# JacobMackay/beifong

Hardware: AMD Instinct MI355X
Metric: Mrays/s (closest + any-hit BVH queries), Bus.obj-class radar scene (higher is better)
Workload: dtype f32

## Files before the change

### beifong_amd/csrc/bf_api.cpp

```cpp
#include <hip/hip_runtime.h>

#include <algorithm>
#include <atomic>
#include <cmath>
#include <cstdarg>
#include <cstdio>
#include <cstring>
#include <limits>
#include <memory>
#include <new>
#include <string>
#include <vector>

#include <dlfcn.h>
#if defined(__has_include) && __has_include(<rccl/rccl.h>)
#include <rccl/rccl.h>
#else
extern "C" {
typedef struct ncclComm *ncclComm_t;
typedef enum { ncclSuccess = 0 } ncclResult_t;
typedef enum { ncclFloat = 7 } ncclDataType_t;
typedef enum { ncclSum = 0 } ncclRedOp_t;
ncclResult_t ncclCommInitAll(ncclComm_t *comm, int ndev, const int *devlist);
ncclResult_t ncclCommDestroy(ncclComm_t comm);
// ... 2616 lines not shown
        if (launch->flags & BF_FLAG_MIX_RESAMPLE) return fail(BF_ERR_INVALID, "BF_FLAG_MIX_RESAMPLE is a receive-mode flag");
        if (is_rx) return fail(BF_ERR_INVALID, "render modes need a sensor (fluxmeter / perspective), not a receiver");
        for (uint32_t i = 0; i < scene->d.n_emitters; ++i)
            if (scene->emitter_types[i] != BF_EMITTER_SPOT && scene->emitter_types[i] != BF_EMITTER_AREA &&
                scene->emitter_types[i] != BF_EMITTER_POINT)
                return fail(BF_ERR_INVALID, "render modes: emitter %u is a transmitter (use receive mode)", i);
    }
    if (launch->mode > BF_MODE_RECEIVE_IQ) return fail(BF_ERR_INVALID, "unknown mode %u", launch->mode);
    if (launch->mode != BF_MODE_RECEIVE_RAW && launch->phase_bins)
        return fail(BF_ERR_INVALID, "phase_bins needs receive mode (PhaseIntegrator wraps pathtimefrequency)");
    if (launch->phase_bins > 4096) return fail(BF_ERR_INVALID, "phase_bins %u out of range", launch->phase_bins);
    if ((launch->mode == BF_MODE_RANGE || launch->mode == BF_MODE_TIME) && (launch->bins == 0 || !(launch->bin_width > 0.f)))
        return fail(BF_ERR_INVALID, "range/time mode needs bins > 0 and bin_width > 0");
    const bool multi_pixel = launch->spp && launch->film_width && launch->film_height;
    if (multi_pixel ? (launch->film_width != scene->film_w || launch->film_height != scene->film_h)
                    : (scene->film_w != 1 || scene->film_h != 1) && !is_rx)
        return fail(BF_ERR_INVALID, "the sensor's film is %u x %u: the launch must name the same film and spp > 0 (it has %u x %u, spp %u)",
                    scene->film_w, scene->film_h, launch->film_width, launch->film_height, launch->spp);
    if (multi_pixel) {
        if (launch->mode == BF_MODE_RECEIVE_RAW || launch->mode == BF_MODE_RECEIVE_IQ)
            return fail(BF_ERR_INVALID, "receive modes bin into the ADC: film_width / film_height / spp must be 0");
        const uint64_t px = (uint64_t) launch->film_width * launch->film_height;
        if (px > (1u << 24) || px * (5ull + 3ull * launch->bins) > (1ull << 31))
            return fail(BF_ERR_UNSUPPORTED, "film %u x %u with %u bins is too large", launch->film_width, launch->film_height, launch->bins);
        if (launch->path_offset + launch->n_paths > px * launch->spp)
            return fail(BF_ERR_INVALID, "path_offset + n_paths = %llu exceeds film_width * film_height * spp = %llu",
                        (unsigned long long) (launch->path_offset + launch->n_paths), (unsigned long long) (px * launch->spp));
    }
    if ((launch->flags & BF_FLAG_MOMENT) && (launch->flags & BF_FLAG_FAST))
        return fail(BF_ERR_INVALID, "BF_FLAG_MOMENT | BF_FLAG_FAST: the fast-arithmetic tolerance contract says nothing about squared "
                                    "samples; render second moments with the exact kernels");
    if (multi_pixel && (launch->flags & BF_FLAG_MOMENT) && (uint64_t) launch->film_width * launch->film_height * (11ull + 6ull * launch->bins) > (1ull << 31))
        return fail(BF_ERR_UNSUPPORTED, "film %u x %u with %u bins and BF_FLAG_MOMENT is too large", launch->film_width, launch->film_height, launch->bins);
    hipStream_t stream = reinterpret_cast<hipStream_t>(stream_);
    const bool rolling = (launch->flags & BF_FLAG_ROLLING) != 0u && launch->n_paths != 0u &&
                         (uint64_t) n_renders * launch->n_paths <= scene->tun.pool && n_renders <= bfd::kRollRing;
    if (launch->flags & BF_FLAG_ROLLING) {
        if (scene->roll.open && ((launch->flags ^ scene->roll.shape.flags) & BF_FLAG_FAST))
            return fail(BF_ERR_INVALID, "BF_FLAG_ROLLING: the open rolling sequence of this handle was started %s BF_FLAG_FAST; "
                                        "flush it (bf_scene_flush) before rolling renders of the other mode",
                        (scene->roll.shape.flags & BF_FLAG_FAST) ? "with" : "without");
        if (scene->roll.open && ((launch->flags ^ scene->roll.shape.flags) & BF_FLAG_MOMENT))
            return fail(BF_ERR_INVALID, "BF_FLAG_ROLLING: the open rolling sequence of this handle was started %s BF_FLAG_MOMENT; "
                                        "flush it (bf_scene_flush) before rolling renders of the other layout",
                        (scene->roll.shape.flags & BF_FLAG_MOMENT) ? "with" : "without");
        if (multi_pixel || (launch->flags & BF_FLAG_MEGAKERNEL))
            return fail(BF_ERR_UNSUPPORTED, "BF_FLAG_ROLLING: multi-pixel films and the one-kernel variant do not roll");
        if (stats_out)
            return fail(BF_ERR_INVALID, "BF_FLAG_ROLLING: a rolling render returns before its paths have ended, so it has no statistics "
                                        "of its own (pass stats_out = NULL; bf_scene_flush reports the sequence's)");
    }
    {
        bf_status ost = order_after_last(scene, stream);
        if (ost != BF_OK) return ost;
        if (!rolling && (ost = close_sequence(scene, stream)) != BF_OK) return ost;
    }
    bfd::DLaunch lp;
    std::memset(&lp, 0, sizeof(lp));
    lp.film_w = multi_pixel ? launch->film_width : 1u;
    lp.film_h = multi_pixel ? launch->film_height : 1u;
    lp.spp = multi_pixel ? launch->spp : 0u;
    lp.mode = launch->mode;
    lp.color_mode = launch->color_mode;
    lp.n_paths = launch->n_paths;
    lp.path_offset = launch->path_offset;
    lp.seed = launch->seed;
    lp.max_depth = launch->max_depth;
    lp.rr_depth = launch->rr_depth;
    lp.bins = launch->bins;
    lp.bins_y = launch->bins_y;
    lp.phase_bins = launch->mode == BF_MODE_RECEIVE_RAW ? launch->phase_bins : 0u;
    lp.iq = launch->mode == BF_MODE_RECEIVE_IQ ? 1u : 0u;
    if (lp.iq) lp.mode = BF_MODE_RECEIVE_RAW;
    lp.bin_width = launch->bin_width;
    lp.time_c = launch->time_c;
    lp.n_chan = bf_launch_channels(launch);
    lp.chan_px = lp.n_chan / (lp.film_w * lp.film_h);
    lp.lean = lean_profile(scene, launch, receive_mode, multi_pixel) ? 1u : 0u;
    lp.wide = scene->sensor_host.filt_n != 0u ? 1u : 0u;
    scene->last_variant = (lp.lean ? (uint32_t) BF_VARIANT_LEAN : 0u) | (lp.wide ? (uint32_t) BF_VARIANT_WIDE : 0u);
    if (launch->flags & BF_FLAG_FAST) scene->last_variant |= (uint32_t) BF_VARIANT_FAST;
    if (launch->flags & BF_FLAG_MOMENT) scene->last_variant |= (uint32_t) BF_VARIANT_MOMENT;
    const Kernels &kern = kernels_for(launch->flags);
    lp.count = ((launch->flags & (BF_FLAG_STATS | BF_FLAG_COUNT)) || stats_out) ? 1u : 0u;
    lp.doppler = (receive_mode && (launch->flags & BF_FLAG_DOPPLER)) ? 1u : 0u;
    lp.resample = (receive_mode && scene->any_resample) ? 1u : 0u;
    if (lp.resample && lp.doppler)
        return fail(BF_ERR_UNSUPPORTED, "BF_FLAG_DOPPLER with a resample_freq transmitter: both rewrite the path's wavelength (one slot of path state)");
    lp.mix = (receive_mode && (launch->flags & BF_FLAG_MIX_RESAMPLE)) ? 1u : 0u;
    lp.n_chan_all = lp.n_chan * n_renders;
    lp.geom_stride = geom_stride;
    lp.lds_hist = (lp.n_chan_all <= (uint32_t) bfd::kMaxLdsHist && !(launch->flags & BF_FLAG_GLOBAL_ATOMICS)) ? 1u : 0u;
    lp.lds_floats = lp.lds_hist ? lp.n_chan_all : 0u;
    size_t lds = sizeof(int) * bfd::kStackDepth * bfd::kBlock + (lp.lds_hist ? sizeof(float) * lp.n_chan_all : 0);
    lds = ((lds + 15) & ~size_t(15)) + (scene->d.tab_cache ? bfd::kTabBytes : 0u);
    if (batch && !rolling) {
        lp.batch = n_renders;
        lp.batch_paths = launch->n_paths;
        lp.n_paths = launch->n_paths * n_renders;
        const size_t seed_bytes = batch->seeds ? ((sizeof(uint64_t) * n_renders + 15) & ~size_t(15)) : 0;
        const size_t off_bytes = batch->mesh_offsets ? sizeof(float4) * n_renders : 0;
        if (seed_bytes + off_bytes) {
            bf_scene::Stage *stg = nullptr;
            bf_status sst = stage_acquire(scene, seed_bytes + off_bytes, &stg);
            if (sst != BF_OK) return sst;
            if (seed_bytes) {
                std::memcpy(stg->host, batch->seeds, sizeof(uint64_t) * n_renders);
                lp.batch_seeds = (const uint64_t *) stg->dev;
            }
            if (off_bytes) {
                float4 *o = (float4 *) ((char *) stg->host + seed_bytes);
                float dmax = 0.f;
                for (uint32_t k = 0; k < n_renders; ++k) {
                    const float *q = batch->mesh_offsets + 3 * k;
                    if (!(std::isfinite(q[0]) && std::isfinite(q[1]) && std::isfinite(q[2])))
                        return fail(BF_ERR_INVALID, "bf_render_batch: non-finite mesh offset of render %u", k);
                    o[k] = make_float4(q[0], q[1], q[2], 0.f);
                    dmax = std::max({dmax, std::fabs(q[0]), std::fabs(q[1]), std::fabs(q[2])});
                }
                if (scene->d.n_tris) {
                    lp.batch_offsets = (const float4 *) ((char *) stg->dev + seed_bytes);
                    lp.box_slack = 1e-6f * (scene->origin_scale_built + 2.f * dmax);
                }
            }
            sst = stage_commit(stg, seed_bytes + off_bytes, stream);
            if (sst != BF_OK) return sst;
        }
    }

    uint64_t want = (lp.n_paths + bfd::kBlock - 1) / bfd::kBlock;
    unsigned blocks_per_cu = (unsigned) std::max<size_t>(1, std::min<size_t>(4, (160 * 1024) / lds));
    unsigned grid = (unsigned) std::max<uint64_t>(1, std::min<uint64_t>(want, (uint64_t) scene->n_cus * blocks_per_cu));

    if (rolling) {
        bf_status rst = wf_roll_render(scene, launch, batch, lp, hist_dev, records_dev, stream);
        if (rst != BF_OK) return rst;
        return mark_last(scene, stream);
    }
    HIP_TRY(hipMemsetAsync(scene->counters, 0, sizeof(unsigned long long) * bfd::CTR_GUARD, stream));
    hipEvent_t ev0 = nullptr, ev1 = nullptr;
    if (stats_out) {
        HIP_TRY(hipEventCreate(&ev0));
        HIP_TRY(hipEventCreate(&ev1));
        HIP_TRY(hipEventRecord(ev0, stream));
    }
    if (launch->n_paths) {
        if (launch->flags & BF_FLAG_MEGAKERNEL) {
            HIP_TRY(kern.render(&scene->d, &lp, hist_dev, records_dev, scene->counters,
                                (launch->flags & BF_FLAG_STATS) ? 1 : 0, grid, lds, stream));
        } else {
            bf_status wst = wf_render(scene, kern, lp, hist_dev, records_dev, stream, (launch->flags & BF_FLAG_STATS) != 0,
                                      stats_out != nullptr);
            if (wst != BF_OK) return wst;
        }
    }
    if (stats_out) {
        HIP_TRY(hipEventRecord(ev1, stream));
        HIP_TRY(hipEventSynchronize(ev1));
        unsigned long long c[bfd::CTR_COUNT];
        HIP_TRY(hipMemcpy(c, scene->counters, sizeof(c), hipMemcpyDeviceToHost));
        if ((launch->flags & BF_FLAG_MEGAKERNEL) || !launch->n_paths) {
            scene->wf_ms[0] = scene->wf_ms[1] = scene->wf_ms[2] = 0.f;
            scene->wf_trace_launches = scene->wf_iters = scene->wf_tail_launches = scene->wf_shade_launches = 0;
        }
        fill_stats(scene, c, lp.n_paths, stats_out);
        float ms = 0.f;
        hipError_t he = hipEventElapsedTime(&ms, ev0, ev1);
// ... 289 lines not shown
                std::memcpy(o, to_world + 12 * r, 12 * sizeof(float));
                o[12] = moves[r] ? 1.f : 0.f;
                o[13] = o[14] = o[15] = 0.f;
            }
        if ((pst = stage_commit(stg, bytes, stream)) != BF_OK) return pst;
        HIP_TRY(bfk_launch_deform_tris(scene->geom->corners, (const bfd::DDeformSrc *) stg->dev, tris0, a + L.tris, normals0,
                                       scene->d.normals ? a + L.normals : nullptr, scene->d.n_tris,
                                       to_world ? (const float *) ((const char *) stg->dev + src_bytes) : nullptr, kc, L.rows, n_shapes * 16u,
                                       bound, scene->deform_bad, stream));
        HIP_TRY(hipEventRecord(stg->ev, stream));
        HIP_TRY(bfk_launch_refit(a + L.tris, nodes0, a + L.nodes, scene->d.qnodes ? a + L.qnodes : nullptr, scene->d.n_nodes, rf.lvl4,
                                 rf.off4.data(), (uint32_t) rf.off4.size() - 1u, a + L.ubox4, wnodes0, scene->d.wnodes ? a + L.wnodes : nullptr,
                                 rf.lvl16, rf.off16.data(), (uint32_t) rf.off16.size() - 1u, a + L.ubox16, 2e-7f * oscale, kc, L.rows, stream));
        return BF_OK;
    });
    if (st != BF_OK || !n_deform) return st;
    if ((st = deform_watch(scene, stream)) != BF_OK) return st;
    return stats_out ? deform_report(scene, true) : BF_OK;
}

bf_status bf_render_device(const bf_scene *scene, const bf_launch *launch, float *hist_dev, bf_path_record *records_dev,
                           void *stream, bf_stats *stats_out) {
    return render_common(scene, launch, nullptr, hist_dev, records_dev, stream, stats_out);
}

bf_status bf_render_batch_device(const bf_scene *scene, const bf_launch *launch, const bf_batch *batch, float *hist_dev,
                                 bf_path_record *records_dev, void *stream, bf_stats *stats_out) {
    if (!batch) return fail(BF_ERR_INVALID, "bf_render_batch_device: null batch");
    return render_common(scene, launch, batch, hist_dev, records_dev, stream, stats_out);
}

bf_status bf_scene_flush(bf_scene *scene, void *stream_, bf_stats *stats_out) {
    if (!scene) return fail(BF_ERR_INVALID, "null argument");
    BF_ENTER(scene);
    hipStream_t stream = reinterpret_cast<hipStream_t>(stream_);
    const bool was_open = scene->roll.open;
    const uint64_t n_paths = was_open ? scene->roll.lp.n_paths : 0;
    bf_status st = order_after_last(scene, stream);
    if (st != BF_OK) return st;
    if (was_open) {
        if ((st = wf_roll_flush(scene, stream, stats_out != nullptr)) != BF_OK) return st;
        if ((st = mark_last(scene, stream)) != BF_OK) return st;
    }
    if (stats_out) {
        std::memset(stats_out, 0, sizeof(*stats_out));
        if (!was_open) return BF_OK;
        HIP_TRY(hipStreamSynchronize(stream));
        unsigned long long c[bfd::CTR_COUNT];
        HIP_TRY(hipMemcpy(c, scene->counters, sizeof(c), hipMemcpyDeviceToHost));
        fill_stats(scene, c, n_paths, stats_out);
        stats_out->kernel_ms = scene->wf_ms[0] + scene->wf_ms[1] + scene->wf_ms[2];
        if (c[bfd::CTR_GUARD] || c[bfd::CTR_SURV_GUARD]) {
            HIP_TRY(hipMemset(scene->counters + bfd::CTR_GUARD, 0, 2 * sizeof(unsigned long long)));
            scene->wf_fb_pending = false;
            return wf_guard_error(c[bfd::CTR_GUARD], c[bfd::CTR_SURV_GUARD]);
        }
        return scene->roll.lp.count ? check_film_count(c, n_paths) : BF_OK;
    }
    return BF_OK;
}

bf_status bf_scene_sync(bf_scene *scene) {
    if (!scene) return fail(BF_ERR_INVALID, "null argument");
    BF_ENTER(scene);
    bf_status st = close_sequence(scene, scene->roll.stream);
    if (st != BF_OK) return st;
    if (scene->has_last) HIP_TRY(hipEventSynchronize(scene->last_done));
    scene->wf_fb_pending = false;
    scene->roll.fb_call_iters = 0;
    unsigned long long lost = 0, refused = 0;
    bf_status gst = read_guards(scene, &lost, &refused);
    if (gst != BF_OK) return gst;
    if (lost || refused) return wf_guard_error(lost, refused);
    return deform_report(scene, true);
}

bf_status bfdbg_preload_guard(bf_scene *scene, unsigned long long n) {
    if (!scene) return fail(BF_ERR_INVALID, "null argument");
    HIP_TRY(hipDeviceSynchronize());
    HIP_TRY(hipMemcpy(scene->counters + bfd::CTR_GUARD, &n, sizeof(n), hipMemcpyHostToDevice));
    return BF_OK;
}

extern "C" hipError_t bfk_gather_probe(int mode, const float4 *table, uint32_t n_rows, float4 *out, hipStream_t stream);
bf_status bfdbg_gather_probe(int mode, uint32_t log2_rows, uint32_t reps, float *ms_out) {
    if (mode < 0 || mode > 2 || log2_rows < 10 || log2_rows > 28 || reps == 0) return fail(BF_ERR_INVALID, "bfdbg_gather_probe: bad arguments");
    const uint32_t n = 1u << log2_rows;
    float4 *table = nullptr, *flush = nullptr, *out = nullptr;
    hipEvent_t e0 = nullptr, e1 = nullptr;
    hipError_t e = hipMalloc((void **) &table, (size_t) n * 16);
    if (e == hipSuccess) e = hipMalloc((void **) &flush, (size_t) n * 16);
    if (e == hipSuccess) e = hipMalloc((void **) &out, 1024 * 16);
    if (e == hipSuccess) e = hipMemset(table, 0, (size_t) n * 16);
    if (e == hipSuccess) e = hipMemset(flush, 0, (size_t) n * 16);
    if (e == hipSuccess) e = hipEventCreate(&e0);
    if (e == hipSuccess) e = hipEventCreate(&e1);
    float total = 0.f;
    for (uint32_t r = 0; r < reps && e == hipSuccess; ++r) {
        e = hipMemsetAsync(flush, (int) (r & 1u), (size_t) n * 16, nullptr);
        if (e == hipSuccess) e = hipEventRecord(e0, nullptr);
        if (e == hipSuccess) e = bfk_gather_probe(mode, table, n, out, nullptr);
        if (e == hipSuccess) e = hipEventRecord(e1, nullptr);
        if (e == hipSuccess) e = hipEventSynchronize(e1);
        float ms = 0.f;
        if (e == hipSuccess) e = hipEventElapsedTime(&ms, e0, e1);
        total += ms;
    }
    if (e0) (void) hipEventDestroy(e0);
    if (e1) (void) hipEventDestroy(e1);
    (void) hipFree(table);
    (void) hipFree(flush);
    (void) hipFree(out);
    if (e != hipSuccess) return fail(BF_ERR_DEVICE, "bfdbg_gather_probe: %s", hipGetErrorString(e));
    if (ms_out) *ms_out = total / (float) reps;
    return BF_OK;
}

bf_status bfdbg_hold_busy(bf_scene *scene, int on) {
    if (!scene) return fail(BF_ERR_INVALID, "null argument");
    if (on) {
        if (scene->busy.test_and_set(std::memory_order_acquire)) return fail(BF_ERR_INVALID, "bfdbg_hold_busy: already held");
    } else {
        scene->busy.clear(std::memory_order_release);
    }
    return BF_OK;
}


void bf_shard_range(uint64_t n_paths, uint32_t shard, uint32_t n_shards, uint64_t *offset, uint64_t *count) {
    if (n_shards == 0) n_shards = 1;
    auto cut = [&](uint64_t k) -> uint64_t { return (uint64_t) (((unsigned __int128) n_paths * k) / n_shards); };
    const uint64_t lo = cut(shard), hi = cut((uint64_t) shard + 1u);
    if (offset) *offset = lo;
    if (count) *count = hi - lo;
}

extern "C++" {
namespace {
struct Rccl {
    void *lib = nullptr;
    decltype(&ncclCommInitAll) comm_init_all = nullptr;
    decltype(&ncclCommDestroy) comm_destroy = nullptr;
    decltype(&ncclAllReduce) all_reduce = nullptr;
    decltype(&ncclGroupStart) group_start = nullptr;
    decltype(&ncclGroupEnd) group_end = nullptr;
    decltype(&ncclGetErrorString) error_string = nullptr;
    std::string why;
};
Rccl &rccl() {
    static Rccl r = [] {
        Rccl q;
        const char *forced = getenv("BF_RCCL_LIB");
        const char *names[] = {forced && *forced ? forced : "librccl.so.1", "librccl.so", "/opt/rocm/lib/librccl.so.1"};
        const size_t n_names = forced && *forced ? 1 : 3;
        for (size_t i = 0; i < n_names && !q.lib; ++i)
            q.lib = dlopen(names[i], RTLD_NOW | RTLD_NOLOAD | RTLD_LOCAL);
        std::string last;
        for (size_t i = 0; i < n_names && !q.lib; ++i) {
            q.lib = dlopen(names[i], RTLD_NOW | RTLD_LOCAL);
            if (!q.lib) {
                const char *e = dlerror();
                last = e ? e : "";
            }
        }
        if (!q.lib) {
            q.why = std::string(forced && *forced ? forced : "librccl.so") + " not found: " + last;
// ... 513 lines not shown
```

### beifong_amd/csrc/bf_device.h

```cpp
#pragma once
#include <hip/hip_runtime.h>

#include "bf_ns.h"
#include <stddef.h>
#include <stdint.h>

#include "../../include/beifong_hip.h"

BF_NS_BEGIN

constexpr uint32_t kTriStride = 3;
constexpr int kBlock = 256;
constexpr int kStackDepth = 32;
constexpr int kMaxLdsHist = 12288;
constexpr int kWideStack = 512;
constexpr uint32_t kTopNodes = 85;

struct DRect {
    float to_world[12];
    float to_object[12];
    float s[3], t[3], n[3];
    float inv_area;
    float area;
    uint32_t shape;
// ... 91 lines not shown

#define BF_CAS __attribute__((address_space(4)))
typedef const BF_CAS DRect CRect;
typedef const BF_CAS DShape CShape;
typedef const BF_CAS DEmitter CEmitter;
typedef const BF_CAS DSensor CSensor;
template <class T> __device__ __forceinline__ const BF_CAS T *as_const(const T *p) { return (const BF_CAS T *) (uintptr_t) p; }
__device__ __forceinline__ CRect *c_rects(const DScene &sc) { return as_const(sc.rects); }
__device__ __forceinline__ CShape *c_shapes(const DScene &sc) { return as_const(sc.shapes); }
__device__ __forceinline__ CEmitter *c_emitters(const DScene &sc) { return as_const(sc.emitters); }
__device__ __forceinline__ CSensor &c_sensor(const DScene &sc) { return *as_const(sc.sensor); }

struct DRoll {
    uint64_t seed, path_offset;
    float *hist;
    bf_path_record *records;
    const DRect *rects;
    const DShape *shapes;
    const DEmitter *emitters;
    const DMaterial *materials;
    const DSensor *sensor;
    float c, lambda_min, lambda_max;
    uint32_t pad;
};
static_assert(sizeof(DRoll) == 88, "descriptor ring entry");
struct DDeformSrc {
    const float *pos;
    const float *nrm;
    uint32_t nv;
    uint32_t pad;
};
static_assert(sizeof(DDeformSrc) == 24, "per-shape table of bf_deform_tris_kernel");

constexpr uint32_t kRollRing = 256;
constexpr uint32_t kRollWindow = 4;
constexpr uint32_t kRollBase = 32;
constexpr uint32_t kRollBaseCh = 5, kRollBaseChMoment = 11;

struct DLaunch {
    uint32_t mode, color_mode;
    uint64_t n_paths, path_offset, seed;
    int32_t max_depth, rr_depth;
    uint32_t bins, bins_y, phase_bins;
    float bin_width, time_c;
    uint32_t n_chan;
    uint32_t lds_hist;
    uint32_t iq;
    uint32_t film_w, film_h;
    uint32_t spp;
    uint32_t chan_px;
    uint32_t batch;
    uint32_t n_chan_all;
    uint64_t batch_paths;
    const uint64_t *batch_seeds;
    const float4 *batch_offsets;
    uint32_t mix;
    uint32_t doppler;
    uint32_t resample;
    float box_slack;
    const DRoll *roll;
    uint32_t roll_newest;
    uint32_t roll_lo;
    uint32_t lds_floats;
    uint32_t base_off;
    uint32_t has_records;
    uint32_t lean;
    uint32_t wide;
    uint32_t multi;
    uint32_t count;
    uint32_t geom_stride;
};

enum {
    CTR_NEXT_PATH = 0, CTR_CLOSEST, CTR_SHADOW, CTR_NODES, CTR_TRIS, CTR_INVALID, CTR_BOUNCES, CTR_TAIL_RAYS, CTR_STARTED, CTR_TRACED,
    CTR_NODES_LDS,
    CTR_TAIL_NODES,
    CTR_TAIL_WNODES,
    CTR_TAIL_TRIS,
    CTR_TAIL_BOUNCES,
    CTR_SHADE_LOADS,
    CTR_SHADE_STORES,
    CTR_SHADE_SHADOW,
    CTR_SHADE_RAYS,
    CTR_FILM,
    CTR_GUARD,
    CTR_SURV_GUARD,
    CTR_COUNT
};

BF_NS_END
```

### beifong_amd/csrc/bf_path_logic.h

```cpp
#pragma once
#include "bf_device_core.h"
#include "bf_wavefront.h"

BF_NS_BEGIN

constexpr uint32_t kFlagValid = 1u << 24, kFlagFilmOk = 1u << 25, kFlagTermPending = 1u << 26, kDepthMask = 0xffffffu;
constexpr uint32_t kFlagFilmLeft = 1u << 27, kFlagFilmUp = 1u << 28;

struct PathState {
    V3 ro, rd;
    float rmint, rmaxt;
    float throughput, eta, emission_weight, result;
    float aux, bs_pdf;
    V3 prev_p;
    uint32_t flags;
    uint32_t n_rays;
    Rng rng;
    uint64_t path_i;
    uint32_t render;
    float time;
    float t_rx;
    float lambda0;
    float phase;
    float dlambda;
};

BF_DEV void load_state(const WF &wf, uint32_t i, bool receive, PathState &s) {
    float4 r0 = wf.ray0(i), r1 = wf.ray1(i), a = wf.sa(i), bb = wf.sb(i);
    uint4 d = wf.sd(i);
    s.ro = mk(r0.x, r0.y, r0.z);
    s.rmint = r0.w;
    s.rd = mk(r1.x, r1.y, r1.z);
    s.rmaxt = r1.w;
    s.throughput = a.x;
    s.eta = a.y;
    s.emission_weight = a.z;
    s.result = a.w;
    s.aux = bb.x;
    s.bs_pdf = bb.y;
    s.prev_p = s.ro;
    s.flags = __float_as_uint(bb.z);
    s.n_rays = __float_as_uint(bb.w);
    s.rng.state = ((uint64_t) d.y << 32) | d.x;
    s.path_i = ((uint64_t) d.w << 32) | d.z;
    s.time = s.t_rx = s.lambda0 = s.phase = 0.f;
    s.render = wf.has_render ? wf.render(i) : 0u;
    s.dlambda = wf.has_dop ? wf.dop(i) : 0.f;
    if (receive) {
        float4 e = wf.se(i);
        s.time = e.x;
        s.t_rx = e.y;
        s.lambda0 = e.z;
        s.phase = e.w;
    }
}
BF_DEV void store_state(const WF &wf, uint32_t j, bool receive, const PathState &s) {
    wf.ray0(j) = make_float4(s.ro.x, s.ro.y, s.ro.z, s.rmint);
    wf.ray1(j) = make_float4(s.rd.x, s.rd.y, s.rd.z, s.rmaxt);
    wf.sa(j) = make_float4(s.throughput, s.eta, s.emission_weight, s.result);
    wf.sb(j) = make_float4(s.aux, s.bs_pdf, __uint_as_float(s.flags), __uint_as_float(s.n_rays));
    wf.sd(j) = make_uint4((uint32_t) s.rng.state, (uint32_t) (s.rng.state >> 32), (uint32_t) s.path_i,
                          (uint32_t) (s.path_i >> 32));
    if (receive) wf.se(j) = make_float4(s.time, s.t_rx, s.lambda0, s.phase);
    if (wf.has_render) wf.render(j) = s.render;
    if (wf.has_dop) wf.dop(j) = s.dlambda;
}
BF_DEV float shape_doppler(const DScene &sc, const SI &si, float lambda_nm) {
    V3 q = xf_point(c_shapes(sc)[si.shape].velocity, to_local(si.sh, si.p));
    return 2.f * dot(si.wi, q) / sc.c * lambda_nm;
}
template <int V> BF_DEV DScene path_scene(const DScene &sc, const DLaunch &lp, uint32_t render) {
    if (!(V & (kMulti | kGeom))) return sc;
    DScene r = sc;
    if (V & kMulti) {
        const BF_CAS DRoll &e = as_const(lp.roll)[render & (kRollRing - 1u)];
        r.rects = e.rects;
        r.shapes = e.shapes;
        r.emitters = e.emitters;
        r.materials = e.materials;
        r.sensor = e.sensor;
        r.c = e.c;
        r.lambda_min = e.lambda_min;
        r.lambda_max = e.lambda_max;
        r.tab_on = 0u;
    }
    if (V & kGeom) geom_version(r, (uint64_t) render * lp.geom_stride);
    return r;
}
BF_DEV Shift path_shift(const DLaunch &lp, uint32_t render) { return make_shift(lp.batch_offsets, render, lp.box_slack); }

BF_DEV uint32_t nth_set_bit(unsigned long long m, uint32_t r) {
    uint32_t pos = 0;
#pragma unroll
    for (int shift = 32; shift >= 1; shift >>= 1) {
        unsigned long long lowmask = (1ull << shift) - 1ull;
        uint32_t cnt = (uint32_t) __popcll(m & lowmask);
        if (r >= cnt) {
            r -= cnt;
            m >>= shift;
            pos += shift;
        } else {
            m &= lowmask;
        }
    }
    return pos;
}

struct MaskCursor {
    const unsigned long long *masks;
    const unsigned long long *masks2;
    uint32_t sel;
    uint32_t b, b_end;
    unsigned long long m;
    uint32_t base, stride;
    uint32_t k;
    unsigned long long sub;
    unsigned long long w;
    unsigned long long nz;
    uint32_t rot, mod, inv, pb;
};
BF_DEV unsigned long long wave_read_u64(unsigned long long v, int src) {
    unsigned lo = (unsigned) __shfl((int) (unsigned) v, src), hi = (unsigned) __shfl((int) (unsigned) (v >> 32), src);
    return ((unsigned long long) hi << 32) | lo;
}
BF_DEV void cursor_fetch(MaskCursor &c, int lane) {
    const uint32_t idx = c.base + (c.k * 64u + (uint32_t) lane) * c.stride;
    uint32_t p = idx + c.rot;
    if (p >= c.mod) p -= c.mod;
    c.w = 0ull;
    if (idx < c.b_end) {
        c.w = c.masks ? c.masks[p] : ~0ull;
        if (c.inv) c.w = ~c.w;
        c.w &= c.sub;
        if (c.sel) c.w &= c.sel == 1u ? c.masks2[p] : ~c.masks2[p];
    }
    c.nz = __ballot(c.w != 0ull);
}
BF_DEV void cursor_seek(MaskCursor &c, int lane) {
    while (true) {
        if (c.nz) {
            const int j = __ffsll((unsigned long long) c.nz) - 1;
            c.nz &= c.nz - 1ull;
            c.b = c.base + (c.k * 64u + (uint32_t) j) * c.stride;
// ... 395 lines not shown
    } while (0)
#else
#define BF_LANEPROF_ARG
#define SLP(sec, cond)
#endif
template <int RX = 2>
BF_DEV bool shade_vertex(const DScene &sc0, const DLaunch &lp, PathState &s, const Hit &hit, ShadowReq &sh,
                         uint32_t &c_bounces BF_SHADEPROF_ARG BF_LANEPROF_ARG) {
    BF_SHADEPROF_STAMP(spf_t0);
    const DScene sc = path_scene<RX>(sc0, lp, s.render);
    const bool receive = mode_receive<RX>(lp);
    const bool is_range = !receive && lp.mode == BF_MODE_RANGE, is_time = rare<RX>(!receive && lp.mode == BF_MODE_TIME);
    const bool iq = receive && lp.iq != 0u;
    const bool phase_bins = rare<RX>(receive && lp.phase_bins != 0u);
    const bool doppler = rare<RX>(receive && lp.doppler != 0u);
    const uint32_t n_emit = (RX & kLean) ? 1u : sc.n_emitters;
    sh.want = false;
    SI si;
    const bool si_valid = hit.t != BF_INF;
    int emitter = -1;
    SLP(10, si_valid);
    bf_material mat;
    mat.type = ~0u;
    mat.back_material = 0u;
    if (si_valid) {
        make_si<false, RX>(sc, s.ro, s.rd, hit, si, nullptr, path_shift(lp, s.render));
        emitter = si.emitter;
        mat = load_material(sc, si.material);
    }
#ifdef BF_VERTEX_PROF
    asm volatile("s_waitcnt vmcnt(0)" ::: "memory");
#endif
    BF_SHADEPROF_STAMP(spf_t1);
    uint32_t depth = s.flags & kDepthMask;
    if (depth == 0) {
        if (si_valid) s.flags |= kFlagValid;
        if (is_range) s.aux += si_valid ? si.t : 0.f;
        if (is_time) s.aux = si_valid ? si.t / lp.time_c : 0.f;
        if (si_valid && doppler) s.dlambda += shape_doppler(sc, si, s.lambda0);
        if (receive && si_valid) {
            s.time += -si.t / sc.c;
            if (phase_bins) s.phase = phase_update(s.phase, -si.t, sc.lambda_min, sc.lambda_max);
        }
        depth = 1;
    } else {
        if (receive) {
            s.time += -hit.t / sc.c;
            if (phase_bins) s.phase = phase_update(0.f, -hit.t, sc.lambda_min, sc.lambda_max);
        }
        SLP(11, emitter >= 0);
        if (emitter >= 0) {
            CEmitter &e = c_emitters(sc)[(RX & kLean) ? 0 : emitter];
            float emitter_pdf = receive ? transmitter_pdf_direction<RX>(sc, e, s.prev_p, si.p, si.sh.n, s.lambda0)
                                        : emitter_pdf_direction<RX>(sc, e, s.prev_p, si.p, si.sh.n);
            if (n_emit != 1) emitter_pdf *= 1.f / (float) n_emit;
            s.emission_weight = mis_weight(s.bs_pdf, emitter_pdf);
        }
        if (is_range) s.aux += si_valid ? si.t : 0.f;
        if (is_time) s.aux += si_valid ? si.t / lp.time_c : 0.f;
        ++depth;
    }
    s.flags = (s.flags & ~kDepthMask) | (depth & kDepthMask);
    SLP(12, emitter >= 0);
    if (emitter >= 0) {
        CEmitter &e = c_emitters(sc)[(RX & kLean) ? 0 : emitter];
        if (doppler) s.dlambda += shape_doppler(sc, si, s.lambda0);
        float ev;
        if (receive)
            ev = transmitter_eval<RX>(sc, e, si, s.time, s.lambda0);
        else
            ev = ((RX & kLean) || e.type == BF_EMITTER_AREA) ? ((si.wi.z > 0.f) ? e.radiance : 0.f) : 0.f;
        float contrib = s.emission_weight * s.throughput * ev;
        if (iq) {
            float re, im;
            path_phasor((s.t_rx - s.time) * sc.c, s.lambda0, re, im);
            s.result += contrib * re;
            s.phase += contrib * im;
        } else {
            s.result += contrib;
        }
        if (is_range) s.aux += si_valid ? si.t : 0.f;
    }
    bool active = si_valid;
    if ((int) depth > lp.rr_depth) {
        float q = __builtin_fminf(s.throughput * sqr(s.eta), .95f);
        active = (next_1d(s.rng) < q) && active;
        s.throughput *= rcp(q);
    }
    if (depth >= (uint32_t) lp.max_depth || !active) return false;

    if (rare<RX>(mat.back_material != 0u) && si.wi.z < 0.f) mat = load_material(sc, mat.back_material - 1u);
    ++c_bounces;
    BF_SHADEPROF_STAMP(spf_t2);
    SLP(13, true);
    SLP(15, mat.type == BF_BSDF_ROUGHCONDUCTOR);
    SLP(16, mat.type != BF_BSDF_ROUGHCONDUCTOR);
    if (bsdf_smooth(mat)) {
        float sx = next_1d(s.rng), sy = next_1d(s.rng);
        DirSample ds;
        ds.d = mk(0, 0, 1);
        ds.pdf = 0.f;
        ds.dist = 0.f;
        ds.delta = false;
        float emitter_val = 0.f;
        if (n_emit >= 1) {
            uint32_t index = 0;
            float emitter_pdf = 1.f;
            if (n_emit > 1) {
                emitter_pdf = 1.f / (float) n_emit;
                index = min((uint32_t) (sx * (float) n_emit), n_emit - 1u);
                sx = (sx - index * emitter_pdf) * (float) n_emit;
            }
            CEmitter &e = c_emitters(sc)[index];
            if (receive)
                emitter_val = transmitter_sample_direction<RX>(sc, e, si.p, s.time, s.lambda0, sx, sy, ds);
            else
                emitter_val = emitter_sample_direction<RX>(sc, e, si.p, sx, sy, ds);
            if (n_emit > 1) {
                ds.pdf *= emitter_pdf;
                emitter_val *= rcp(emitter_pdf);
            }
        }
        SLP(14, ds.pdf != 0.f);
        if (ds.pdf != 0.f) {
            V3 wo = to_local(si.sh, ds.d);
            float bsdf_val, bsdf_pdf;
            bsdf_eval_pdf(mat, si.wi, wo, bsdf_val, bsdf_pdf);
            float mis = ds.delta ? 1.f : mis_weight(ds.pdf, bsdf_pdf);
            sh.c = mis * s.throughput * bsdf_val * emitter_val;
            sh.c_im = 0.f;
            if (iq) {
                float re, im;
                path_phasor((s.t_rx - s.time) * sc.c + ds.dist, s.lambda0, re, im);
                sh.c_im = sh.c * im;
                sh.c = sh.c * re;
            }
            sh.o = si.p;
            sh.d = ds.d;
            sh.mint = kRayEpsilon * (1.f + hmax_abs(si.p));
            sh.maxt = ds.dist * (1.f - kShadowEpsilon);
            sh.want = true;
            ++s.n_rays;
        }
        if (is_range) s.aux += si.t;
    }
    BF_SHADEPROF_STAMP(spf_t3);
    (void) next_1d(s.rng);
    float s2x = next_1d(s.rng), s2y = next_1d(s.rng);
    BSDFSample bs;
    float bsdf_val = bsdf_sample(mat, si.wi, s2x, s2y, bs);
    s.throughput = s.throughput * bsdf_val;
    if (s.throughput == 0.f) {
        s.flags |= kFlagTermPending;
        s.rmint = BF_INF;
        s.rmaxt = 0.f;
        return true;
    }
    s.eta *= bs.eta;
    s.ro = si.p;
    s.rd = to_world(si.sh, bs.wo);
    s.rmint = (1.f + hmax_abs(si.p)) * kRayEpsilon;
    s.rmaxt = BF_INF;
    s.prev_p = si.p;
    s.bs_pdf = bs.pdf;
    ++s.n_rays;
#ifdef BF_VERTEX_PROF
    if (spf) {
// ... 520 lines not shown
```

### beifong_amd/csrc/bf_wavefront.h

```cpp
#pragma once
#include <hip/hip_runtime.h>

#include "bf_ns.h"
#include <stddef.h>
#include <stdint.h>

BF_NS_BEGIN

constexpr uint32_t kWfMaxIter = 4096;
constexpr uint32_t kShadeChain = 8;
constexpr uint32_t kTraceRefill = 32;
constexpr uint32_t kTraceStragglers = 12;
constexpr uint32_t kTraceBlocksPerCU = 8;
constexpr uint32_t kTailSmallPool = 1u << 22;
constexpr uint32_t kTailRowJobs = 12;

#define BF_HD __host__ __device__ __forceinline__

struct WF {
    float4 *recA, *recB, *recC;
    BF_HD float4 &ray0(uint32_t i) const { return recA[4 * (size_t) i + 0]; }
    BF_HD float4 &ray1(uint32_t i) const { return recA[4 * (size_t) i + 1]; }
    BF_HD float4 &hit(uint32_t i) const { return recA[4 * (size_t) i + 2]; }
    BF_HD uint32_t &hit_prim(uint32_t i) const { return reinterpret_cast<uint32_t *>(recA + 4 * (size_t) i + 3)[0]; }
    BF_HD uint32_t &render(uint32_t i) const { return reinterpret_cast<uint32_t *>(recA + 4 * (size_t) i + 3)[1]; }
    BF_HD float &dop(uint32_t i) const { return reinterpret_cast<float *>(recA + 4 * (size_t) i + 3)[2]; }
    BF_HD float4 &sa(uint32_t i) const { return recB[4 * (size_t) i + 0]; }
    BF_HD float4 &sb(uint32_t i) const { return recB[4 * (size_t) i + 1]; }
    BF_HD uint4 &sd(uint32_t i) const { return reinterpret_cast<uint4 *>(recB)[4 * (size_t) i + 2]; }
    BF_HD float4 &se(uint32_t i) const { return recB[4 * (size_t) i + 3]; }
    BF_HD float4 &sh0(uint32_t i) const { return recC[4 * (size_t) i + 0]; }
    BF_HD float4 &sh1(uint32_t i) const { return recC[4 * (size_t) i + 1]; }
    BF_HD float &sh2(uint32_t i) const { return reinterpret_cast<float *>(recC + 4 * (size_t) i + 2)[0]; }
    BF_HD float &sh3(uint32_t i) const { return reinterpret_cast<float *>(recC + 4 * (size_t) i + 2)[1]; }
    uint32_t has_render;
    uint32_t has_dop;
    const float4 *offsets;
    float box_slack;
    uint32_t geom_stride;
    unsigned long long *m_alive[2];
    unsigned long long *m_trace[2];
    unsigned long long *m_shadow[2];
    unsigned long long *m_hit[2];
    uint32_t hit_split;
    uint32_t chain_min;
    uint32_t reserved[3];
    uint32_t *n_live;
    unsigned long long *counters;
    uint32_t trace_refill, trace_stragglers;
    uint32_t iq;
    uint32_t shade_chain;
    uint32_t row_jobs;
    uint32_t n_slots;
    uint32_t capacity;
    uint32_t n_main, n_surv;
    uint32_t *surv_cursor;
    uint32_t wake_b0, wake_nb;
    uint32_t tail_share;
    uint32_t surv_claims_max;
};
static_assert(sizeof(WF) == 216 && offsetof(WF, n_live) == 136, "WF is a kernel argument: its layout is the kernels' argument layout");

BF_NS_END
```

### beifong_amd/csrc/bf_wavefront.hip

```cpp
#include "bf_path_logic.h"

BF_NS_BEGIN

BF_DEV void publish_masks(unsigned long long *m_out, bool aligned, bool merge, uint32_t batch0, uint32_t slot, bool valid_lane, bool bit) {
    if (aligned) {
        unsigned long long w = __ballot(bit);
        if ((threadIdx.x & 63) == 0 && w) {
            if (merge)
                atomicOr(&m_out[batch0], w);
            else
                m_out[batch0] = w;
        }
    } else if (valid_lane && bit) {
        atomicOr(&m_out[slot >> 6], 1ull << (slot & 63u));
    }
}

BF_DEV bool presolve_ray(const DScene &sc, bool any, V3 o, V3 d, float mint, float maxt, Hit &best, bool &found, const Shift &shf) {
    best.t = BF_INF;
    best.u = best.v = 0.f;
    best.prim = 0;
    best.slot = 0;
    found = false;
    for (uint32_t i = 0; i < sc.n_rects; ++i) {
// ... 71 lines not shown
#endif
template <int FIRST, int W, int RX>
__global__ __launch_bounds__(kBlock, W) void wf_shade(DScene sc_arg, DLaunch lp, WF wf, uint32_t it, float *__restrict__ g_hist,
                                                      bf_path_record *__restrict__ records) {
    extern __shared__ __align__(16) unsigned char s_raw[];
    float *s_hist = reinterpret_cast<float *>(s_raw);
    const int tid = threadIdx.x, lane = tid & 63;
    DScene sc = sc_arg;
    if (RX & kMulti) sc.tab_cache = 0u;
    load_tables_lds(sc, (4u * lp.lds_floats + 15u) & ~15u, (uint32_t) tid);
    constexpr bool WALK = FIRST == 0 || FIRST == 3;
    constexpr bool EVICT = FIRST == 3;
    const bool lds_hist = lp.lds_hist != 0;
    if (lp.lds_floats || sc.tab_on) {
        for (uint32_t i = tid; i < lp.lds_floats; i += kBlock) s_hist[i] = 0.f;
        __syncthreads();
    }
    const int cur = it & 1, nxt = cur ^ 1;
    const bool receive = mode_receive<RX>(lp);
    if (FIRST == 2 && blockIdx.x == 0 && tid == 0) {
        wf.surv_cursor[0] += wf.surv_cursor[1];
        wf.surv_cursor[1] = 0u;
    }
    const uint32_t n_batches = WALK ? wf.n_slots >> 6 : (FIRST == 2 ? wf.wake_nb : wf.n_main >> 6);
    unsigned long long *m_alive = wf.m_alive[nxt], *m_trace = wf.m_trace[nxt], *m_shadow = wf.m_shadow[nxt], *m_hit = wf.m_hit[nxt];
    SurvAlloc sv = {0ull, 0u, 0u, EVICT ? wf.surv_cursor[0] : 0u};

    FilmAcc acc = {0.f, 0.f, 0.f, 0.f, 0.f, 0u, 0u};
    uint32_t c_closest = 0, c_shadow = 0, c_bounces = 0, c_live = 0, c_traced = 0, c_loads = 0, c_shq = 0;
#ifdef BF_SHADE_PROF
    const bool lpf = BF_SHADE_PROF >= 2;
    ShadeProf spf = {0, 0, 0, 0};
    unsigned long long t_sec[8] = {0, 0, 0, 0, 0, 0, 0, 0};
    unsigned long long slt_last = __builtin_amdgcn_s_memtime();
#endif

    const uint32_t n_waves = gridDim.x * (kBlock / 64), wave_id = blockIdx.x * (kBlock / 64) + (tid >> 6);
    MaskCursor cur_alive;
    const uint32_t n_pass = (WALK && wf.hit_split) ? 2u : 1u;
    uint32_t first_b = wave_id;
    const bool rolling = lp.roll != nullptr;

    for (uint32_t pass = 0; pass < n_pass; ++pass) {
    if (WALK) cursor_init(cur_alive, wf.m_alive[cur], wave_id, n_waves, n_batches, lane, 1u, n_pass == 2u ? wf.m_hit[cur] : nullptr, pass ? 1u : 2u);
    while (true) {
        uint32_t slot = 0, got;
        bool aligned;
        if (!WALK) {
            if (first_b >= n_batches) break;
            uint32_t fb = first_b;
            if (FIRST == 2) {
                fb += wf.wake_b0;
                if (fb >= wf.n_main >> 6) fb -= wf.n_main >> 6;
            }
            slot = fb * 64u + lane;
            got = 64;
            aligned = true;
            first_b += n_waves;
        } else {
            cursor_skip_empty(cur_alive, lane);
            if (cursor_empty(cur_alive)) break;
            const uint32_t batch_before = cur_alive.b;
            const bool whole = __popcll(cur_alive.m) == 64;
            got = cursor_take(cur_alive, 64u, true, (uint32_t) lane, slot, lane);
            if (got == 0) break;
            aligned = whole && got == 64 && slot == batch_before * 64u + (uint32_t) lane;
            aligned = __all(aligned);
        }
        bool has = (uint32_t) lane < got;
        const uint32_t batch0 = slot >> 6;
        if (FIRST == 2) has = ((m_alive[batch0] >> lane) & 1ull) == 0ull;

        PathState s;
        s.render = 0u;
        ShadowReq sh;
        sh.want = false;
        bool need_gen = false, cont = false, have_hit = false;
        Hit hit;
        hit.t = BF_INF;
        hit.u = hit.v = 0.f;
        hit.prim = 0;
        hit.slot = 0;

        SLP(0, has);
        SLT(0);
        if (has) {
            if (!WALK) {
                need_gen = true;
                s.path_i = (uint64_t) slot - (uint64_t) wf.n_main;
                if (FIRST == 2) {
                    const uint4 d = wf.sd(slot);
                    s.path_i = ((uint64_t) d.w << 32) | d.z;
                }
            } else {
                load_state(wf, slot, receive, s);
                ++c_loads;
                SLP(1, (s.flags & kFlagTermPending) != 0);
                if (s.flags & kFlagTermPending) {
                    film_put<RX>(sc, lp, s, s_hist, g_hist, lds_hist, acc, records);
                    need_gen = true;
                } else {
                    float4 hq = wf.hit(slot);
                    hit.t = hq.x;
                    hit.u = hq.y;
                    hit.v = hq.z;
                    hit.slot = __float_as_int(hq.w);
                    have_hit = true;
                }
            }
        }
#ifdef BF_SHADE_PROF
        asm volatile("s_waitcnt vmcnt(0)" ::: "memory");
#endif
        SLT(1);
        bool settled = !has;
        bool touched = FIRST != 2;
        bool tracing = false, shadowing = false;
        for (uint32_t round = 0;; ++round) {
            SLP(2 + min(round, 2u), !settled && have_hit);
            if (!settled && have_hit) {
                have_hit = false;
#ifdef BF_SHADE_PROF
                cont = shade_vertex<RX>(sc, lp, s, hit, sh, c_bounces, &spf, lpf);
#else
                cont = shade_vertex<RX>(sc, lp, s, hit, sh, c_bounces);
#endif
                SLT(7);
                SLP(5, !cont);
                if (!cont) {
                    film_put<RX>(sc, lp, s, s_hist, g_hist, lds_hist, acc, records);
                    need_gen = true;
                } else if (!(s.flags & kFlagTermPending)) {
                    ++c_closest;
                }
                if (sh.want) ++c_shadow;
            }
            SLT(2);
            SLP(6, !settled && need_gen);
            if (!settled && need_gen) {
                need_gen = false;
                cont = false;
                const uint64_t path_i = s.path_i + wf.n_main;
                if (slot < wf.n_main && path_i < lp.n_paths) {
                    touched = true;
                    generate_path<RX>(sc, lp, path_i, s);
                    sh.want = false;
                    ++c_closest;
                    cont = true;
                }
            }
            SLT(3);
            if (!settled) {
                tracing = cont && !(s.flags & kFlagTermPending);
                shadowing = cont && sh.want;
                const Shift shf = path_shift(lp, s.render);
                const DScene scp = path_scene<RX>(sc, lp, s.render);
                SLP(7, shadowing);
                SLP(8, tracing);
                if (shadowing) {
                    Hit tmp;
                    bool found;
                    if (!presolve_ray(scp, true, sh.o, sh.d, sh.mint, sh.maxt, tmp, found, shf)) {
                        s.result += found ? sh.c * 0.f : sh.c;
                        if (receive && lp.iq) s.phase += found ? sh.c_im * 0.f : sh.c_im;
                        shadowing = false;
                    }
                    sh.want = shadowing;
                }
                if (tracing) {
                    bool found;
                    tracing = presolve_ray(scp, false, s.ro, s.rd, s.rmint, s.rmaxt, hit, found, shf);
                }
            }
            SLT(4);
            const bool resolved = !settled && cont && !tracing && !shadowing;
            const bool real_hit = !(s.flags & kFlagTermPending) && hit.t != BF_INF;
            const bool lonely = wf.chain_min != 0u && (uint32_t) __popcll(__ballot(resolved && real_hit)) < wf.chain_min;
            const bool chain = resolved && round + 1u < wf.shade_chain && !(lonely && real_hit);
            if (!__any(chain)) break;
            SLP(9, chain && (s.flags & kFlagTermPending));
            SLP(17 + min(round, 2u), chain);
            if (chain) {
                if (s.flags & kFlagTermPending) {
                    film_put<RX>(sc, lp, s, s_hist, g_hist, lds_hist, acc, records);
                    need_gen = true;
                    cont = false;
                } else {
                    have_hit = true;
                }
            } else {
                settled = true;
// ... 165 lines not shown
                    } else {
                        r0 = wf.ray0(slot);
                        r1 = wf.ray1(slot);
                        any = false;
                    }
                    o = mk(r0.x, r0.y, r0.z);
                    d = mk(r1.x, r1.y, r1.z);
                    mint = r0.w;
                    maxt = r1.w;
                    found = false;
                    has = true;
                    best.t = BF_INF;
                    best.u = best.v = 0.f;
                    best.prim = 0;
                    best.slot = 0;
                    if (!phase_shadow) {
                        float4 hq = wf.hit(slot);
                        best.t = hq.x;
                        best.u = hq.y;
                        best.v = hq.z;
                        best.slot = __float_as_int(hq.w);
                        best.prim = wf.hit_prim(slot);
                    }
                    if (GEOM) grows = (uint64_t) wf.render(slot) * wf.geom_stride;
                    if (SHIFT) {
                        shf = make_shift(wf.offsets, wf.render(slot), wf.box_slack);
                        ray_inverse_shift(o, d, shf, id, oid, ohi);
                    } else {
                        ray_inverse(o, d, id, oid);
                    }
                    node = sc.root;
                    st.sp = 0;
                }
                served += got;
                want -= got;
                if (want && cursor_empty(cursor) && phase_shadow) {
                    phase_shadow = false;
                    cursor_init(cursor, wf.m_trace[nxt], wave_id, n_waves, n_batches, lane);
                }
            }
        }
        if (__ballot(has) == 0ull) break;
        guard = 0;

        while (true) {
            if (++guard > kTraceGuard) {
                const unsigned long long lost = __ballot(has);
                if (lane == 0) atomicAdd(&wf.counters[CTR_GUARD], (unsigned long long) __popcll(lost));
                has = false;
                break;
            }
            while (true) {
                const unsigned long long at_node = __ballot(has && node >= 0);
                if (!at_node) break;
                if ((uint32_t) __popcll(at_node) < wf.trace_stragglers && __ballot(has && node < 0 && node != kNoNode)) break;
                if (has && node >= 0) {
                    if (STATS) {
                        ++c_nodes;
                        c_top += node < n_top ? 1u : 0u;
                    }
                    if (QUANT)
                        node = node4q_step_top(GEOM ? sc.qnodes + grows : sc.qnodes, s_top, n_top, node, id, oid, SHIFT ? ohi : oid, mint,
                                               any ? maxt : __builtin_fminf(maxt, best.t), st);
                    else
                        node = node4_step_top(GEOM ? sc.nodes + grows : sc.nodes, s_top, n_top, node, id, oid, SHIFT ? ohi : oid, mint,
                                              any ? maxt : __builtin_fminf(maxt, best.t), st);
                }
            }
            if (has && node < 0 && node != kNoNode) {
                if (GEOM) {
                    DScene scg = sc;
                    scg.tris += grows;
                    found = leaf_intersect<STATS>(scg, node, any, o, d, mint, maxt, best, c_tris);
                } else {
                    found = SHIFT ? leaf_intersect<STATS>(sc, node, any, o, d, mint, maxt, best, c_tris, shf)
                                  : leaf_intersect<STATS>(sc, node, any, o, d, mint, maxt, best, c_tris);
                }
                node = found ? kNoNode : st.pop_or_none();
            }
            if (has && node == kNoNode) {
                if (any) {
                    const float c = wf.sh2(job);
                    if (!found || !__builtin_isfinite(c)) {
                        float4 a = wf.sa(job);
                        a.w += found ? c * 0.f : c;
                        wf.sa(job) = a;
                    }
                    if (wf.iq) {
                        const float ci = wf.sh3(job);
                        if (!found || !__builtin_isfinite(ci)) {
                            float4 e = wf.se(job);
                            e.w += found ? ci * 0.f : ci;
                            wf.se(job) = e;
                        }
                    }
                } else {
                    wf.hit(job) = make_float4(best.t, best.u, best.v, __int_as_float(best.slot));
                    if (wf.hit_split && best.t != BF_INF) atomicOr(&wf.m_hit[nxt][job >> 6], 1ull << (job & 63u));
                }
                has = false;
            }
            unsigned long long act = __ballot(has);
            if (act == 0ull) break;
            if (work_left() && (uint32_t) __popcll(act) <= wf.trace_refill) break;
        }
    }
    if (STATS) {
        unsigned long long v_nodes = c_nodes, v_tris = c_tris, v_top = c_top;
#pragma unroll
        for (int off = 32; off > 0; off >>= 1) {
            v_nodes += __shfl_down(v_nodes, off);
            v_tris += __shfl_down(v_tris, off);
            v_top += __shfl_down(v_top, off);
        }
        if (lane == 0) {
            atomicAdd(&wf.counters[CTR_NODES], v_nodes);
            atomicAdd(&wf.counters[CTR_TRIS], v_tris);
            atomicAdd(&wf.counters[CTR_NODES_LDS], v_top);
        }
    }
}

BF_NS_END

#ifdef BF_SHADE_PROF
extern "C" int bfdbg_shade_lane_profile(unsigned long long *out, int clear) {
    if (hipDeviceSynchronize() != hipSuccess) return -1;
    if (out && hipMemcpyFromSymbol(out, HIP_SYMBOL(bfd::g_lane_prof), sizeof(unsigned long long) * 2 * bfd::kShadeProfSections) != hipSuccess) return -1;
    if (clear) {
        void *p = nullptr;
        if (hipGetSymbolAddress(&p, HIP_SYMBOL(bfd::g_lane_prof)) != hipSuccess) return -1;
        if (hipMemset(p, 0, sizeof(unsigned long long) * 2 * bfd::kShadeProfSections) != hipSuccess) return -1;
    }
    return 2 * bfd::kShadeProfSections;
}
#endif

static hipError_t wf_shade_launch(const bfd::DScene *sc, const bfd::DLaunch *lp, const bfd::WF *wf, uint32_t it, int first,
                                  float *g_hist, bf_path_record *records, unsigned grid, size_t lds_bytes,
                                  hipStream_t stream, int waves, bool moment) {
    const bool rx = lp->mode == BF_MODE_RECEIVE_RAW;
#define BF_SHADE_LAUNCH_RX(F, W, RX_)                                                                                              \
    hipLaunchKernelGGL((bfd::wf_shade<F, W, RX_>), dim3(grid), dim3(bfd::kBlock), lds_bytes, stream, *sc, *lp, *wf, it, g_hist, records)
#define BF_SHADE_LAUNCH(F, W)            \
    if (rx) BF_SHADE_LAUNCH_RX(F, W, 1); \
    else BF_SHADE_LAUNCH_RX(F, W, 0)
#define BF_SHADE_LAUNCH_WIDE(F)                          \
    if (rx) BF_SHADE_LAUNCH_RX(F, 3, 1 | bfd::kWide);    \
    else BF_SHADE_LAUNCH_RX(F, 3, 0 | bfd::kWide)
#define BF_SHADE_LAUNCH_LEAN(F)                          \
    if (rx) BF_SHADE_LAUNCH_RX(F, 3, 1 | bfd::kLean);    \
    else BF_SHADE_LAUNCH_RX(F, 3, 0 | bfd::kLean)
#define BF_SHADE_LAUNCH_MULTI(F)                         \
    if (rx) BF_SHADE_LAUNCH_RX(F, 3, 1 | bfd::kMulti);   \
    else BF_SHADE_LAUNCH_RX(F, 3, 0 | bfd::kMulti)
#define BF_SHADE_LAUNCH_GEOM(F, V)                           \
    if (rx) BF_SHADE_LAUNCH_RX(F, 3, 1 | bfd::kGeom | (V));  \
    else BF_SHADE_LAUNCH_RX(F, 3, 0 | bfd::kGeom | (V))
#define BF_SHADE_LAUNCH_GEOM_V(F)                                          \
    if (lp->lean && !lp->wide) { BF_SHADE_LAUNCH_GEOM(F, bfd::kLean); }    \
    else if (lp->wide) { BF_SHADE_LAUNCH_GEOM(F, bfd::kWide); }            \
    else { BF_SHADE_LAUNCH_GEOM(F, 0); }
#if !BF_FAST
#define BF_SHADE_LAUNCH_MOM(F, V)                                \
    if (rx) BF_SHADE_LAUNCH_RX(F, 3, 1 | bfd::kMoment | (V));    \
    else BF_SHADE_LAUNCH_RX(F, 3, 0 | bfd::kMoment | (V))
#define BF_SHADE_LAUNCH_MOM_F(V)                         \
    if (first == 3) { BF_SHADE_LAUNCH_MOM(3, V); }       \
    else if (first == 2) { BF_SHADE_LAUNCH_MOM(2, V); }  \
// ... 138 lines not shown
```

Measured before the change: 1672.

## Split path state into hot and cold loads, skip cold reload on misses

Reorders the per-path state record so the fields needed on every shade visit (aux, result, flags, rng, path index) sit together. The cold ray and throughput fields are now loaded only when the path has a real hit and is not terminating. The result accumulator moves from sa to sb, and the any-hit shadow accumulation is updated to match. The diff also adds optional per-category shade-visit counters behind a stats level, and skips the Russian-roulette RNG draw for inactive paths, which may change the RNG sequence. The intent is less global memory traffic per shade visit when many rays miss or terminate.

```diff
diff --git a/beifong_amd/csrc/bf_api.cpp b/beifong_amd/csrc/bf_api.cpp
--- a/beifong_amd/csrc/bf_api.cpp
+++ b/beifong_amd/csrc/bf_api.cpp
@@ -2722,7 +2722,7 @@
     if (launch->flags & BF_FLAG_FAST) scene->last_variant |= (uint32_t) BF_VARIANT_FAST;
     if (launch->flags & BF_FLAG_MOMENT) scene->last_variant |= (uint32_t) BF_VARIANT_MOMENT;
     const Kernels &kern = kernels_for(launch->flags);
-    lp.count = ((launch->flags & (BF_FLAG_STATS | BF_FLAG_COUNT)) || stats_out) ? 1u : 0u;
+    lp.count = (launch->flags & BF_FLAG_STATS) ? 2u : (((launch->flags & BF_FLAG_COUNT) || stats_out) ? 1u : 0u);
     lp.doppler = (receive_mode && (launch->flags & BF_FLAG_DOPPLER)) ? 1u : 0u;
     lp.resample = (receive_mode && scene->any_resample) ? 1u : 0u;
     if (lp.resample && lp.doppler)
@@ -3178,6 +3178,14 @@
     return BF_OK;
 }
 
+bf_status bfdbg_shade_visits(bf_scene *scene, unsigned long long *out) {
+    if (!scene || !out) return fail(BF_ERR_INVALID, "null argument");
+    HIP_TRY(hipDeviceSynchronize());
+    HIP_TRY(hipMemcpy(out, scene->counters + bfd::CTR_SHADE_TERM, 3 * sizeof(unsigned long long), hipMemcpyDeviceToHost));
+    return BF_OK;
+}
+static_assert(bfd::CTR_SHADE_MISS == bfd::CTR_SHADE_TERM + 1 && bfd::CTR_SHADE_FULL == bfd::CTR_SHADE_TERM + 2, "read as one block");
+
 extern "C" hipError_t bfk_gather_probe(int mode, const float4 *table, uint32_t n_rows, float4 *out, hipStream_t stream);
 bf_status bfdbg_gather_probe(int mode, uint32_t log2_rows, uint32_t reps, float *ms_out) {
     if (mode < 0 || mode > 2 || log2_rows < 10 || log2_rows > 28 || reps == 0) return fail(BF_ERR_INVALID, "bfdbg_gather_probe: bad arguments");
diff --git a/beifong_amd/csrc/bf_device.h b/beifong_amd/csrc/bf_device.h
--- a/beifong_amd/csrc/bf_device.h
+++ b/beifong_amd/csrc/bf_device.h
@@ -197,6 +197,9 @@
     CTR_SHADE_STORES,
     CTR_SHADE_SHADOW,
     CTR_SHADE_RAYS,
+    CTR_SHADE_TERM,
+    CTR_SHADE_MISS,
+    CTR_SHADE_FULL,
     CTR_FILM,
     CTR_GUARD,
     CTR_SURV_GUARD,
diff --git a/beifong_amd/csrc/bf_path_logic.h b/beifong_amd/csrc/bf_path_logic.h
--- a/beifong_amd/csrc/bf_path_logic.h
+++ b/beifong_amd/csrc/bf_path_logic.h
@@ -25,20 +25,11 @@
     float dlambda;
 };
 
-BF_DEV void load_state(const WF &wf, uint32_t i, bool receive, PathState &s) {
-    float4 r0 = wf.ray0(i), r1 = wf.ray1(i), a = wf.sa(i), bb = wf.sb(i);
+BF_DEV void load_state_hot(const WF &wf, uint32_t i, bool receive, PathState &s) {
+    float4 bb = wf.sb(i);
     uint4 d = wf.sd(i);
-    s.ro = mk(r0.x, r0.y, r0.z);
-    s.rmint = r0.w;
-    s.rd = mk(r1.x, r1.y, r1.z);
-    s.rmaxt = r1.w;
-    s.throughput = a.x;
-    s.eta = a.y;
-    s.emission_weight = a.z;
-    s.result = a.w;
     s.aux = bb.x;
-    s.bs_pdf = bb.y;
-    s.prev_p = s.ro;
+    s.result = bb.y;
     s.flags = __float_as_uint(bb.z);
     s.n_rays = __float_as_uint(bb.w);
     s.rng.state = ((uint64_t) d.y << 32) | d.x;
@@ -54,11 +45,27 @@
         s.phase = e.w;
     }
 }
+BF_DEV void load_state_cold(const WF &wf, uint32_t i, PathState &s) {
+    float4 r0 = wf.ray0(i), r1 = wf.ray1(i), a = wf.sa(i);
+    s.ro = mk(r0.x, r0.y, r0.z);
+    s.rmint = r0.w;
+    s.rd = mk(r1.x, r1.y, r1.z);
+    s.rmaxt = r1.w;
+    s.throughput = a.x;
+    s.eta = a.y;
+    s.emission_weight = a.z;
+    s.bs_pdf = a.w;
+    s.prev_p = s.ro;
+}
+BF_DEV void load_state(const WF &wf, uint32_t i, bool receive, PathState &s) {
+    load_state_hot(wf, i, receive, s);
+    load_state_cold(wf, i, s);
+}
 BF_DEV void store_state(const WF &wf, uint32_t j, bool receive, const PathState &s) {
     wf.ray0(j) = make_float4(s.ro.x, s.ro.y, s.ro.z, s.rmint);
     wf.ray1(j) = make_float4(s.rd.x, s.rd.y, s.rd.z, s.rmaxt);
-    wf.sa(j) = make_float4(s.throughput, s.eta, s.emission_weight, s.result);
-    wf.sb(j) = make_float4(s.aux, s.bs_pdf, __uint_as_float(s.flags), __uint_as_float(s.n_rays));
+    wf.sa(j) = make_float4(s.throughput, s.eta, s.emission_weight, s.bs_pdf);
+    wf.sb(j) = make_float4(s.aux, s.result, __uint_as_float(s.flags), __uint_as_float(s.n_rays));
     wf.sd(j) = make_uint4((uint32_t) s.rng.state, (uint32_t) (s.rng.state >> 32), (uint32_t) s.path_i,
                           (uint32_t) (s.path_i >> 32));
     if (receive) wf.se(j) = make_float4(s.time, s.t_rx, s.lambda0, s.phase);
@@ -620,7 +627,7 @@
         if (is_range) s.aux += si_valid ? si.t : 0.f;
     }
     bool active = si_valid;
-    if ((int) depth > lp.rr_depth) {
+    if (active && (int) depth > lp.rr_depth) {
         float q = __builtin_fminf(s.throughput * sqr(s.eta), .95f);
         active = (next_1d(s.rng) < q) && active;
         s.throughput *= rcp(q);
diff --git a/beifong_amd/csrc/bf_wavefront.h b/beifong_amd/csrc/bf_wavefront.h
--- a/beifong_amd/csrc/bf_wavefront.h
+++ b/beifong_amd/csrc/bf_wavefront.h
@@ -25,9 +25,9 @@
     BF_HD uint32_t &hit_prim(uint32_t i) const { return reinterpret_cast<uint32_t *>(recA + 4 * (size_t) i + 3)[0]; }
     BF_HD uint32_t &render(uint32_t i) const { return reinterpret_cast<uint32_t *>(recA + 4 * (size_t) i + 3)[1]; }
     BF_HD float &dop(uint32_t i) const { return reinterpret_cast<float *>(recA + 4 * (size_t) i + 3)[2]; }
-    BF_HD float4 &sa(uint32_t i) const { return recB[4 * (size_t) i + 0]; }
-    BF_HD float4 &sb(uint32_t i) const { return recB[4 * (size_t) i + 1]; }
-    BF_HD uint4 &sd(uint32_t i) const { return reinterpret_cast<uint4 *>(recB)[4 * (size_t) i + 2]; }
+    BF_HD float4 &sb(uint32_t i) const { return recB[4 * (size_t) i + 0]; }
+    BF_HD uint4 &sd(uint32_t i) const { return reinterpret_cast<uint4 *>(recB)[4 * (size_t) i + 1]; }
+    BF_HD float4 &sa(uint32_t i) const { return recB[4 * (size_t) i + 2]; }
     BF_HD float4 &se(uint32_t i) const { return recB[4 * (size_t) i + 3]; }
     BF_HD float4 &sh0(uint32_t i) const { return recC[4 * (size_t) i + 0]; }
     BF_HD float4 &sh1(uint32_t i) const { return recC[4 * (size_t) i + 1]; }
diff --git a/beifong_amd/csrc/bf_wavefront.hip b/beifong_amd/csrc/bf_wavefront.hip
--- a/beifong_amd/csrc/bf_wavefront.hip
+++ b/beifong_amd/csrc/bf_wavefront.hip
@@ -177,6 +177,8 @@
         hit.prim = 0;
         hit.slot = 0;
 
+        bool term = false, full = false;
+
         SLP(0, has);
         SLT(0);
         if (has) {
@@ -188,20 +190,33 @@
                     s.path_i = ((uint64_t) d.w << 32) | d.z;
                 }
             } else {
-                load_state(wf, slot, receive, s);
+                load_state_hot(wf, slot, receive, s);
+                const float4 hq = wf.hit(slot);
+                hit.t = hq.x;
+                hit.u = hq.y;
+                hit.v = hq.z;
+                hit.slot = __float_as_int(hq.w);
                 ++c_loads;
-                SLP(1, (s.flags & kFlagTermPending) != 0);
-                if (s.flags & kFlagTermPending) {
-                    film_put<RX>(sc, lp, s, s_hist, g_hist, lds_hist, acc, records);
-                    need_gen = true;
-                } else {
-                    float4 hq = wf.hit(slot);
-                    hit.t = hq.x;
-                    hit.u = hq.y;
-                    hit.v = hq.z;
-                    hit.slot = __float_as_int(hq.w);
-                    have_hit = true;
-                }
+                term = (s.flags & kFlagTermPending) != 0;
+                full = !term && hit.t != BF_INF;
+                if (full) load_state_cold(wf, slot, s);
+            }
+        }
+        if (WALK && lp.count >= 2u) {
+            const unsigned long long bt = __ballot(term), bf = __ballot(full), bm = __ballot(has) & ~(bt | bf);
+            if (lane == 0) {
+                if (bt) atomicAdd(&wf.counters[CTR_SHADE_TERM], (unsigned long long) __popcll(bt));
+                if (bm) atomicAdd(&wf.counters[CTR_SHADE_MISS], (unsigned long long) __popcll(bm));
+                if (bf) atomicAdd(&wf.counters[CTR_SHADE_FULL], (unsigned long long) __popcll(bf));
+            }
+        }
+        if (WALK && has) {
+            SLP(1, term);
+            if (term) {
+                film_put<RX>(sc, lp, s, s_hist, g_hist, lds_hist, acc, records);
+                need_gen = true;
+            } else {
+                have_hit = true;
             }
         }
 #ifdef BF_SHADE_PROF
@@ -533,9 +548,9 @@
                 if (any) {
                     const float c = wf.sh2(job);
                     if (!found || !__builtin_isfinite(c)) {
-                        float4 a = wf.sa(job);
-                        a.w += found ? c * 0.f : c;
-                        wf.sa(job) = a;
+                        float4 a = wf.sb(job);
+                        a.y += found ? c * 0.f : c;
+                        wf.sb(job) = a;
                     }
                     if (wf.iq) {
                         const float ci = wf.sh3(job);
```

Result: no change. 1668 (-0.3%).
